# LeiXu84/fireFoam-dev

Measured on AMD Instinct MI355X. Metric: PIMPLE outer-iterations/sec on 64M-cell hex mesh; pEqn SpMV GB/s vs HBM peak, higher is better.
Workload: dtype f64; 1 GPU; synthetic 400^3 hex box (64000000 cells), buoyant plume + 5-species EDC-shaped source, PIMPLE 1/2/0: rhoEqn + UEqn + YEEqn(4 Yi + h) + 2 pEqn per step; cells=64000000, faces=191520000, parallelism=1 GPU, transport_solvers=PBiCGStab+DILU

## Files before the change

firefoam-dev_amd/binding.py:

```python
import ctypes as C
import os
import re
import subprocess

import numpy as np

_HERE = os.path.dirname(os.path.abspath(__file__))
_ROOT = os.path.dirname(_HERE)
_SO = os.path.join(_HERE, "lib", "libffm.so")
_HDR = os.path.join(_ROOT, "include", "ffm.h")

SOLVERS = {"PCG": 0, "PBiCGStab": 1, "PBiCG": 2, "diagonal": 3, "smoothSolver": 4}
PRECONDS = {"none": 0, "DIC": 1, "DILU": 2, "GaussSeidel": 3, "symGaussSeidel": 4, "diagonal": 5}


class FfmError(RuntimeError):
    pass


class Perf(C.Structure):
    _fields_ = [("initialResidual", C.c_double), ("finalResidual", C.c_double),
                ("nIterations", C.c_int), ("converged", C.c_int), ("singular", C.c_int)]

    def as_dict(self):
# ... 260 lines not shown
        "ffm_flow_order_create_staged": ([vp, C.POINTER(vp)], C.c_int),
        "ffm_flow_order_nstages": ([vp], C.c_int),
        "ffm_solve_ordered_staged_d": ([vp, vp, dp, dp, C.POINTER(Perf)], C.c_int),
        "ffm_plume_set_initial_state": ([vp, C.POINTER(C.c_void_p), hp, hp, hp, C.c_double], C.c_int),
        "ffm_plume_override_mv_weights": ([vp, hp], C.c_int),
        "ffm_plume_ncells": ([vp], C.c_int),
        "ffm_plume_nfaces": ([vp], C.c_int),
        "ffm_plume_get_field": ([vp, C.c_char_p, hp], C.c_int),
        "ffm_plume_nsolves": ([vp], C.c_int),
        "ffm_plume_joint_steps": ([vp], C.c_int),
        "ffm_plume_get_solve": ([vp, C.c_int, C.c_char_p, C.POINTER(Perf)], C.c_int),
        "ffm_plume_get_raw": ([vp, C.c_char_p, hp, C.c_long], C.c_long),
        "ffm_plume_ldu": ([vp], vp),
        "ffm_plume_mesh": ([vp], vp),
        "ffm_fv_multivariate_weights_tiled": ([vp, C.c_int, C.POINTER(C.c_int), C.c_double, C.c_double, C.c_double, dp] + [C.POINTER(C.c_void_p)] * 2 + [dp], C.c_int),
        "ffm_comm_unique_id": ([vp], C.c_int),
        "ffm_comm_init": ([vp, C.c_int, C.c_int, vp], C.c_int),
        "ffm_comm_init_host": ([vp, C.c_int, C.c_int, vp, HOST_ALLREDUCE_FN, HOST_EXCHANGE_FN], C.c_int),
        "ffm_comm_set_host_exchange2": ([vp, HOST_EXCHANGE2_FN], C.c_int),
        "ffm_plume_create_block": ([vp, C.c_int, C.c_int, C.c_int, ip, ip, ip, C.c_double, C.c_double, C.POINTER(vp)], C.c_int),
        "ffm_ldu_create_hint": ([vp, C.c_int, C.c_int, C.c_int, ip, ip, ip, C.POINTER(vp)], C.c_int),
        "ffm_renumber_hint": ([C.c_int, C.c_int, C.c_int, ip, ip, ip, ip, ip], C.c_int),
        "ffm_ldu_create_ext": ([vp, C.c_int, C.c_int, C.c_int, ip, ip, C.POINTER(vp)], C.c_int),
        "ffm_renumber_levels_ext": ([C.c_int, C.c_int, C.c_int, ip, ip, ip, ip], C.c_int),
        "ffm_ldu_check_layout": ([C.c_int, C.c_int, C.c_int, ip, ip], C.c_int),
        "ffm_ldu_set_ghost_exchange": ([vp, C.c_int, ip, ip, ip, ip], C.c_int),
        "ffm_halo_refresh_d": ([vp, dp], C.c_int),
        "ffm_ldu_nowned": ([vp], C.c_int),
        "ffm_comm_rank": ([vp], C.c_int),
        "ffm_comm_size": ([vp], C.c_int),
# ... 923 lines not shown
```

firefoam-dev_amd/csrc/ffm_fused.hip:

```cpp
#include "ffm_mesh.hpp"

constexpr int FUSE_MAX = 5;
constexpr int FUSE_MAX_OWN = 4;
#define CHECK_M(m) if (!(m)) { ffm_set_error("null mesh"); return FFM_ERR_ARG; }

struct GradMulti {
    const double *vf[FUSE_MAX], *vb[FUSE_MAX];
    double *gx[FUSE_MAX], *gy[FUSE_MAX], *gz[FUSE_MAX];
};

template <int W, int NF>
__global__ __launch_bounds__(256) void k_grad_multi(MeshView q, GradMulti a)
{
    CELL_SCHED(ci, q) {
        const int c = (int)ci;
        RowEnt<W> L, U; load_lower<W>(q.v, c, L); load_upper<W>(q.v, c, U);
        double wl[W], wu[W], sx[2 * W], sy[2 * W], sz[2 * W];
#pragma unroll
        for (int s = 0; s < W; s++) {
            wl[s] = q.w[L.f[s]]; wu[s] = q.w[U.f[s]];
            sx[s] = q.Sfx[L.f[s]]; sy[s] = q.Sfy[L.f[s]]; sz[s] = q.Sfz[L.f[s]];
            sx[W + s] = q.Sfx[U.f[s]]; sy[W + s] = q.Sfy[U.f[s]]; sz[W + s] = q.Sfz[U.f[s]];
        }
        const double V = q.V[c];
// ... 212 lines not shown
                        const int n = U.nb[s];
                        const double l = mv_limiter(sch, a.twoByk, a.lo, a.hi, fl[CH + s], vc, vf[n], dx[CH + s] * a.gx[i][n] + dy[CH + s] * a.gy[i][n] + dz[CH + s] * a.gz[i][n]);
                        lim[CH + s] = i == 0 ? l : fmin(lim[CH + s], l);
                    }
                }
            }
#pragma unroll
            for (int s = 0; s < CH; s++) {
                if (mine[s]) { const int e = L.f[s]; const double p0 = fl[s] >= 0 ? 1.0 : 0.0; a.out[e] = lim[s] * q.w[e] + (1.0 - lim[s]) * p0; }
                if (mine[CH + s] || ghostUp[s]) { const int e = U.f[s]; const double p0 = fl[CH + s] >= 0 ? 1.0 : 0.0; a.out[e] = lim[CH + s] * q.w[e] + (1.0 - lim[CH + s]) * p0; }
            }
        }
    }
}

constexpr int MVT_ENT = 256, MVT_FLD = 6, MVT_RUN = 32;
struct MvTile {
    const double *vf[MVT_FLD], *vb[MVT_FLD];
    int scheme[MVT_FLD], nf;
    const double *phi, *Cx, *Cy, *Cz;
    double twoByk, lo, hi;
    double *out;
    const int4 *seg, *rec;
};
template <int W>
__global__ __launch_bounds__(256) void k_mv_tile(MeshView q, MvTile a)
{
    __shared__ double ring[MVT_FLD][3 * MVT_ENT];
    __shared__ int4 shRec[3];
    const int4 sg = a.seg[blockIdx.x];
    const int gBeg = sg.x, ea = sg.y, eb = sg.z, gEnd = sg.w;
    const int t = threadIdx.x;
    const int nf = a.nf;
    auto stage = [&](int ee) {
        if (ee < gBeg || ee >= gEnd) { if (t == 0) shRec[(ee + 3) % 3] = make_int4(0, 0, 0, 0); return; }
        const int4 R = a.rec[ee];
        const int c0 = R.x, cnt = R.y & 0xFFFF;
        if (t == 0) shRec[ee % 3] = make_int4(c0, cnt, 0, 0);
        if (t < cnt) {
            const int c = c0 + t, o = (ee % 3) * MVT_ENT + t;
            for (int i = 0; i < nf; i++) ring[i][o] = a.vf[i][c];
        }
    };
    stage(ea - 1); stage(ea);
    for (int ee = ea; ee < eb; ee++) {
        stage(ee + 1);
        __syncthreads();
        const int4 Rm = shRec[(ee + 2) % 3], R0 = shRec[ee % 3], Rp = shRec[(ee + 1) % 3];
// ... 16 lines not shown
            }
            double gcur[2 * W];
#pragma unroll
            for (int s = 0; s < 2 * W; s++) gcur[s] = a.vf[0][gn[s]];
#pragma unroll
            for (int s = 0; s < W; s++) {
                fl[s] = L.on[s] ? a.phi[L.f[s]] : 0.0; mine[s] = L.on[s] && !(fl[s] > 0);
                fl[W + s] = U.on[s] ? a.phi[U.f[s]] : 0.0; mine[W + s] = U.on[s] && fl[W + s] > 0;
                lim[s] = lim[W + s] = 1.0;
                wl[s] = q.w[L.f[s]]; wu[s] = q.w[U.f[s]];
                sx[s] = q.Sfx[L.f[s]]; sy[s] = q.Sfy[L.f[s]]; sz[s] = q.Sfz[L.f[s]];
                sx[W + s] = q.Sfx[U.f[s]]; sy[W + s] = q.Sfy[U.f[s]]; sz[W + s] = q.Sfz[U.f[s]];
            }
#pragma unroll
            for (int s = 0; s < W; s++) {
                dx[s] = cx - a.Cx[L.nb[s]]; dy[s] = cy - a.Cy[L.nb[s]]; dz[s] = cz - a.Cz[L.nb[s]];
                dx[W + s] = a.Cx[U.nb[s]] - cx; dy[W + s] = a.Cy[U.nb[s]] - cy; dz[W + s] = a.Cz[U.nb[s]] - cz;
            }
            const double V = q.V[c];
            const int j = q.cellB[c];
#pragma unroll 1
            for (int i = 0; i < nf; i++) {
                const double P = ring[i][own];
                double vl[W], vu[W], gnext[2 * W];
                const double *__restrict__ vfn = a.vf[i + 1 < nf ? i + 1 : i];
#pragma unroll
                for (int s = 0; s < 2 * W; s++) gnext[s] = vfn[gn[s]];
#pragma unroll
                for (int s = 0; s < W; s++) {
                    const int k = sl[s] >= 0 ? sl[s] : own, ku = sl[W + s] >= 0 ? sl[W + s] : own;
                    const double rl = ring[i][k], ru = ring[i][ku];
                    vl[s] = sl[s] >= 0 ? rl : gcur[s]; vu[s] = sl[W + s] >= 0 ? ru : gcur[W + s];
// ... 3 lines not shown
                for (int s = 0; s < W; s++) if (L.on[s]) {
                    const double ff = wl[s] * vl[s] + (1.0 - wl[s]) * P;
                    ax -= sx[s] * ff; ay -= sy[s] * ff; az -= sz[s] * ff;
                }
#pragma unroll
                for (int s = 0; s < W; s++) if (U.on[s]) {
                    const double ff = wu[s] * P + (1.0 - wu[s]) * vu[s];
                    ax += sx[W + s] * ff; ay += sy[W + s] * ff; az += sz[W + s] * ff;
                }
                if (j >= 0) for (int tt = q.bcStart[j]; tt < q.bcStart[j + 1]; tt++) {
                    const int k = q.bcItem[tt]; const double b = a.vb[i][k];
                    ax += q.bSfx[k] * b; ay += q.bSfy[k] * b; az += q.bSfz[k] * b;
                }
                const double gxc = ax / V, gyc = ay / V, gzc = az / V;
                const int sch = a.scheme[i];
#pragma unroll
                for (int s = 0; s < W; s++) {
                    if (mine[s]) {
                        const double l = mv_limiter(sch, a.twoByk, a.lo, a.hi, fl[s], vl[s], P, dx[s] * gxc + dy[s] * gyc + dz[s] * gzc);
                        lim[s] = i == 0 ? l : fmin(lim[s], l);
                    }
                    if (mine[W + s]) {
                        const double l = mv_limiter(sch, a.twoByk, a.lo, a.hi, fl[W + s], P, vu[s], dx[W + s] * gxc + dy[W + s] * gyc + dz[W + s] * gzc);
                        lim[W + s] = i == 0 ? l : fmin(lim[W + s], l);
                    }
                }
#pragma unroll
                for (int s = 0; s < 2 * W; s++) gcur[s] = gnext[s];
            }
#pragma unroll
            for (int s = 0; s < W; s++) {
                if (mine[s]) { const int e = L.f[s]; const double p0 = fl[s] >= 0 ? 1.0 : 0.0; a.out[e] = lim[s] * q.w[e] + (1.0 - lim[s]) * p0; }
                if (mine[W + s]) { const int e = U.f[s]; const double p0 = fl[W + s] >= 0 ? 1.0 : 0.0; a.out[e] = lim[W + s] * q.w[e] + (1.0 - lim[W + s]) * p0; }
            }
        }
        __syncthreads();
    }
}

extern "C" int ffm_fv_multivariate_weights_tiled(ffm_mesh *m, int nf, const int *schemes, double k, double lo, double hi, const double *phi_f,
                                                 const double *const *vf, const double *const *vb, double *out_w)
{
    CHECK_M(m);
    if (nf < 1 || !schemes || !phi_f || !vf || !vb || !out_w) return FFM_ERR_ARG;
    FfmFvSegs sg;
    if (nf > MVT_FLD || m->A->maxW > 3 || !ffm_tile_fv_segments(m->A, MVT_RUN, &sg)) return FFM_ERR_UNSUPPORTED;
    MvTile a;
    for (int i = 0; i < MVT_FLD; i++) {
        const int qq = i < nf ? i : 0;
        if (i < nf && ((schemes[qq] != 2 && schemes[qq] != 3) || !vf[qq] || (m->B && !vb[qq]))) return FFM_ERR_ARG;
        a.vf[i] = vf[qq]; a.vb[i] = vb[qq]; a.scheme[i] = schemes[qq];
    }
    a.nf = nf; a.phi = phi_f; a.Cx = m->C[0]; a.Cy = m->C[1]; a.Cz = m->C[2]; a.twoByk = 2.0 / std::max(k, 1e-15); a.lo = lo; a.hi = hi; a.out = out_w;
    a.seg = sg.seg; a.rec = sg.rec;
    hipLaunchKernelGGL(k_mv_tile<3>, dim3(sg.nSeg), dim3(256), 0, m->ctx->stream, mview(m), a);
    FFM_HIP(hipGetLastError());
    return FFM_OK;
}

struct LustSource {
    const double *gx[3], *gy[3], *gz[3], *U0[3];
    double *src[3];
    const double *phi, *rho0, *Cx, *Cy, *Cz, *Cfx, *Cfy, *Cfz;
    double rdt;
};

template <int W>
__global__ __launch_bounds__(256) void k_lust_source(MeshView q, LustSource a)
{
    CELL_SCHED(ci, q) {
// ... 67 lines not shown
            const double w = limited_weight(a.scheme, a.twoByk, a.lo, a.hi, fl[s], wl[s], kl[s], P, dlx[s], dly[s], dlz[s], glx[s], gly[s], glz[s]);
            const double Kf = w * kl[s] + (1.0 - w) * P;
            acc = acc - fl[s] * Kf;
        }
#pragma unroll
        for (int s = 0; s < W; s++) if (U.on[s]) {
            const double w = limited_weight(a.scheme, a.twoByk, a.lo, a.hi, fu[s], wu[s], P, ku[s], dux[s], duy[s], duz[s], gux[s], guy[s], guz[s]);
            const double Kf = w * P + (1.0 - w) * ku[s];
            acc += fu[s] * Kf;
        }
        const int j = q.cellB[c];
        if (j >= 0) for (int t = q.bcStart[j]; t < q.bcStart[j + 1]; t++) { const int k = q.bcItem[t]; acc += a.phib[k] * a.Kb[k]; }
        a.divK[c] = acc / q.V[c];
        a.ddtK[c] = a.rdt * (a.rho[c] * P - a.rho0[c] * a.K0[c]);
        a.ndpdt[c] = -a.dpdt[c];
    }
}


extern "C" int ffm_fvc_grad_multi(ffm_mesh *m, int nf, const double *const *vf, const double *const *vb, double *const *gx,
                                  double *const *gy, double *const *gz)
{
    CHECK_M(m);
    if (nf < 1 || nf > FUSE_MAX_OWN || !vf || !vb || !gx || !gy || !gz) return FFM_ERR_ARG;
    GradMulti a;
    for (int i = 0; i < FUSE_MAX; i++) { const int k = i < nf ? i : 0; a.vf[i] = vf[k]; a.vb[i] = vb[k]; a.gx[i] = gx[k]; a.gy[i] = gy[k]; a.gz[i] = gz[k]; }
    for (int i = 0; i < nf; i++) if (!vf[i] || (m->B && !vb[i]) || !gx[i] || !gy[i] || !gz[i]) return FFM_ERR_ARG;
#define GM(NF) FFM_DISPATCH_W(m->A->maxW, LAUNCH_CELLS((k_grad_multi<W, NF>), mview(m), a))
    switch (nf) { case 1: GM(1); break; case 2: GM(2); break; case 3: GM(3); break; default: GM(4); break; }
#undef GM
// ... 169 lines not shown
    CHECK_M(m);
    if ((scheme != 2 && scheme != 3) || !phi_f || !K || !gx || !gy || !gz || !rho || !rho0 || !K0 || !dpdt || !divK || !ddtK || !negDpdt) return FFM_ERR_ARG;
    if (m->B && (!phi_b || !K_b)) return FFM_ERR_ARG;
    DivPhiK a;
    a.K = K; a.Kb = K_b; a.gx = gx; a.gy = gy; a.gz = gz; a.phi = phi_f; a.phib = phi_b; a.rho = rho; a.rho0 = rho0; a.K0 = K0; a.dpdt = dpdt;
    a.Cx = m->C[0]; a.Cy = m->C[1]; a.Cz = m->C[2]; a.divK = divK; a.ddtK = ddtK; a.ndpdt = negDpdt;
    a.rdt = rDeltaT; a.twoByk = 2.0 / std::max(k, 1e-15); a.lo = lo; a.hi = hi; a.scheme = scheme;
    if (m->A->maxW > 8) return FFM_ERR_UNSUPPORTED;
    if (m->A->maxW <= 3) LAUNCH_CELLS(k_div_phiK<3>, mview(m), a);
    else if (m->A->maxW <= 4) LAUNCH_CELLS(k_div_phiK<4>, mview(m), a);
    else LAUNCH_CELLS(k_div_phiK<8>, mview(m), a);
    FFM_HIP(hipGetLastError());
    return FFM_OK;
}

struct HbyA3 {
    const double *upper, *lower, *src[3], *ic[3], *bc[3], *psi[3], *rAU;
    double *out[3];
};
template <int W>
__global__ __launch_bounds__(256) void k_matrix_HbyA3(MeshView q, HbyA3 a)
{
    CELL_SCHED(ci, q) {
        const int c = (int)ci;
        RowEnt<W> L, U; load_lower<W>(q.v, c, L); load_upper<W>(q.v, c, U);
        double al[W], au[W];
#pragma unroll
        for (int s = 0; s < W; s++) { al[s] = a.lower[L.f[s]]; au[s] = a.upper[U.f[s]]; }
        double bd[3] = {0.0, 0.0, 0.0}, bda = 0.0, bs[3] = {0.0, 0.0, 0.0};
        const int j = q.cellB[c];
// ... 696 lines not shown
```

firefoam-dev_amd/csrc/ffm_plume.hip:

```cpp
#include "ffm_plume.hpp"

static int hydrostatic_init(ffm_plume *P)
{
    ffm_mesh *m = P->mesh; const int N = P->N, B = P->B;
    double *ph = P->ph_rgh, *rhof = P->wF[0], *sg = P->wF[1], *phig = P->wF[2], *rhob = P->wB[0], *fTop = P->wB[1], *div = P->wN[0];
    const double *gh = P->gh, *ghf = P->ghf, *magSf = ffm_mesh_geom(m, 1);
    double *p = P->p, *rho = P->rho; const double *psi = P->psi;
    const double *kind = P->kind_d;
    forN(P, B, [=] __device__(long k) { fTop[k] = (kind[k] > 1.5 && kind[k] < 2.5) ? 1.0 : 0.0; });
    forN(P, N, [=] __device__(long i) { p[i] = ph[i] + rho[i] * gh[i] + PREF; });
    FFM_TRY(thermo_correct(P)); mul(P, rho, psi, p, N);
    const long nNat = P->nNat;
    for (int corr = 0; corr < 5; corr++) {
        FFM_TRY(ffm_fvc_interpolate(m, nullptr, rho, rhof));
        zg(P, rhob, rho);
        FFM_TRY(ffm_fvc_snGrad(m, rho, sg));
        forN(P, nNat, [=] __device__(long e) { phig[e] = -rhof[e] * ghf[e] * sg[e] * magSf[e]; });
        FFM_TRY(ffm_fvm_transport(m, 0.0, nullptr, nullptr, nullptr, rhof, +1, P->diag, P->upper, P->lower));
        FFM_TRY(ffm_fvm_boundary_coeffs(m, nullptr, rhob, +1, fTop, P->zeroB, P->zeroB, P->ic[0], P->bc[0]));
        FFM_TRY(ffm_fvc_surface_integrate(m, phig, P->zeroB, div));
        {
            double *s0 = P->src[0]; const double *dv = div, *V = ffm_mesh_geom(m, 0);
            forN(P, N, [=] __device__(long i) { s0[i] = V[i] * dv[i]; });
        }
// ... 191 lines not shown
    P->fP = dalloc(P, B); P->refP = dalloc(P, B); P->gradP = dalloc(P, B); P->zeroB = dalloc(P, B);
    P->oneB = dupload(P, std::vector<double>(std::max(B, 1), 1.0));
    P->diag = NN(); P->upper = dalloc(P, nNat); P->lower = dalloc(P, nNat); P->dWork = NN(); P->sWork = NN();
    P->Udiag = NN(); P->Uupper = dalloc(P, nNat); P->Ulower = dalloc(P, nNat);
    for (int c = 0; c < 3; c++) { P->src[c] = NN(); P->ic[c] = dalloc(P, B); P->bc[c] = dalloc(P, B); P->Usrc[c] = NN(); P->Uic[c] = dalloc(P, B); P->Ubc[c] = dalloc(P, B); }
    for (auto &w : P->wN) w = NN();
    for (auto &w : P->wF) w = dalloc(P, nNat);
    P->ddtCorrF = dalloc(P, nNat);
    for (auto &w : P->wB) w = dalloc(P, B);
    for (int c = 0; c < 3; c++) { P->UdW[c] = NN(); P->UsW[c] = NN(); P->Ub[c] = P->wB[1 + c]; }
    P->wFuel = P->wN[8]; P->Qdot = P->wN[9]; P->Yt = P->wN[10]; P->alphaEff_f = P->wF[0]; P->alphaEff_b = P->wB[4];
    const bool fused = P->fused = getenv("FFM_PLUME_UNFUSED") == nullptr;
    P->mvSelection = getenv("FFM_PLUME_INDEPENDENT_LIMITERS") == nullptr;
    { const char *e = getenv("FFM_PLUME_SEPARATE_H"); P->separateH = e && atoi(e) != 0; }
    if (P->mvSelection) { P->wMv = dalloc(P, nNat); if (fused) for (int j = 0; j < 2; j++) for (int d = 0; d < 3; d++) P->mvG[j][d] = NN(); }
    for (int j = 0; j < 4; j++) {
        for (int d = 0; d < 3; d++) P->gM[j][d] = fused ? NN() : nullptr;
        P->spD[j] = fused ? NN() : nullptr; P->spS[j] = fused ? NN() : nullptr; P->suM[j] = fused ? NN() : nullptr;
        const bool ownOffDiag = fused && (j == 0 || !P->mvSelection);
        P->spU[j] = ownOffDiag ? dalloc(P, nNat) : nullptr; P->spL[j] = ownOffDiag ? dalloc(P, nNat) : nullptr; P->spB[j] = (fused || P->mvSelection) ? dalloc(P, B) : nullptr;
    }
    for (double *p : P->pool) if (!p) { ffm_set_error("plume: out of device memory"); return FFM_ERR_HIP; }
    PL_HIP(hipDeviceSynchronize());
    delete tmS_; tmS_ = new FfmStageTimer("plume_create: hydrostatic init");
    standin_thermo(P);
    mul(P, P->rho, P->psi, P->p, N);
    FFM_TRY(hydrostatic_init(P));
    PL_HIP(hipStreamSynchronize(ctx->stream));
    delete tmS_; tmS_ = nullptr;
    if (const char *e = getenv("FFM_PLUME_RADIATION")) { if (atoi(e) > 0) FFM_TRY(ffm_plume_set_radiation(P, atoi(e), 2, 4, nullptr, nullptr)); }
// ... 306 lines not shown
```

firefoam-dev_amd/csrc/ffm_plume.hpp:

```cpp
#pragma once
#include "ffm_internal.hpp"
#include "ffm_device.hpp"
#include <algorithm>
#include <cmath>
#include <string>

namespace {
constexpr double RR = 8314.47, CP = 1005.0, TREF = 298.15, PREF = 101325.0, MU = 1.8e-5, PR = 0.7;
constexpr double S_O2 = 3.6282945, HC = 46357151.0, TAU = 0.05, T_IN = 600.0, U_IN = 0.5, SIGMA_SB = 5.670367e-8;
constexpr int NSP = 5, INERT = 4;
const double WMOL[NSP] = {31.9988, 18.0153, 44.0962, 44.01, 28.0134};
const double Y_AMB[NSP] = {0.23301, 0.0, 0.0, 0.0, 0.76699};
const double Y_IN[NSP] = {0.0, 0.0, 1.0, 0.0, 0.0};
const double NU[NSP] = {-S_O2, 4 * 18.0153 / 44.0962, -1.0, 3 * 44.01 / 44.0962, 0.0};
const char *const SPN[NSP] = {"O2", "H2O", "C3H8", "CO2", "N2"};
enum { P_INLET = 0, P_FLOOR = 1, P_TOP = 2, P_SIDES = 3 };

template <class F> __global__ void k_for(long n, F f)
{
    for (long i = (long)blockIdx.x * blockDim.x + threadIdx.x; i < n; i += (long)gridDim.x * blockDim.x) f(i);
}
}

struct SolveLog { char name[16]; ffm_perf perf; };
// ... 9 lines not shown
    double hAmb = 0.0;
    std::vector<double *> pool;
    double *Y[NSP], *Y0[NSP], *T, *hs, *hs0, *U[3], *U0[3], *p, *p0, *p_rgh, *p_rgh0, *psi, *psi0, *rho, *rho0, *K, *K0, *dpdt;
    double *phi, *phib, *gh, *ghf, *ph_rgh, *ph_rgh_b;
    double *kind_d;
    double *fU[3], *refU[3], *fS, *refS, *fP, *refP, *gradP, *zeroB, *oneB;
    double *fStaticU[3], *fStaticS, *fStaticH, *fH, *refY[NSP], *refH;
    double *diag, *upper, *lower, *src[3], *ic[3], *bc[3], *dWork, *sWork;
    double *UdW[3], *UsW[3];
    double *wN[12], *wF[6], *wB[8];
    double *wFuel, *Qdot, *Yt, *alphaEff_f, *alphaEff_b, *Ub[3];
    double *ddtCorrF = nullptr; bool ddtCorrValid = false;
    double *gM[4][3], *spD[4], *spU[4], *spL[4], *spS[4], *spB[4], *suM[4];
    bool mvSelection = true;
    double *wMv = nullptr, *mvG[2][3] = {{nullptr, nullptr, nullptr}, {nullptr, nullptr, nullptr}};
    bool fused = true;
    bool separateH = false;
    int jointSteps = 0;
    double *Udiag, *Uupper, *Ulower, *Usrc[3], *Uic[3], *Ubc[3];
    std::vector<SolveLog> log;
    bool tight = false;
    int stepNo = 0, radFreq = 0;
    std::vector<double> rayD, rayOmega;
    std::vector<int> hL2, hU2, hOldToNew; std::vector<signed char> hFd2;
    int *radCm[3] = {nullptr, nullptr, nullptr}, *radFm[3] = {nullptr, nullptr, nullptr};
    double *radDB = nullptr, *radSB = nullptr, *radPsiB = nullptr, *radUB = nullptr, *radLB = nullptr;
    bool radOrdered = false;
    int radOrdering = 0; bool radMaps = false, radStaged = false;
    int nbrRank[6] = {-1, -1, -1, -1, -1, -1}, gOff[7] = {0, 0, 0, 0, 0, 0, 0}, blkGrid[3] = {1, 1, 1}, blkAt[3] = {0, 0, 0};
    int *radHaloCells = nullptr; int nRadHaloCells = 0; double *radGhostBuf = nullptr;
// ... 125 lines not shown
```

firefoam-dev_amd/csrc/ffm_plume_step.hip:

```cpp
#include "ffm_plume.hpp"

static void bc_update_f(ffm_plume *P, double *f, const double *fStatic)
{ const double *pb = P->phib; forN(P, P->B, [=] __device__(long k) { f[k] = fStatic[k] < 0 ? 1.0 - (pb[k] >= 0 ? 1.0 : 0.0) : fStatic[k]; }); }

static int update_bcs(ffm_plume *P)
{
    for (int c = 0; c < 3; c++) bc_update_f(P, P->fU[c], P->fStaticU[c]);
    bc_update_f(P, P->fS, P->fStaticS);
    bc_update_f(P, P->fH, P->fStaticH);
    return FFM_OK;
}

static int U_boundary(ffm_plume *P)
{
    for (int c = 0; c < 3; c++) FFM_TRY(ffm_bc_values(P->mesh, P->fU[c], P->refU[c], P->zeroB, P->U[c], P->Ub[c]));
    return FFM_OK;
}

static int bc_p_rgh(ffm_plume *P, const double *grad , const double *rhob)
{
    const double *kind = P->kind_d, *pb = P->phib, *phb = P->ph_rgh_b;
    const double *u0 = P->Ub[0], *u1 = P->Ub[1], *u2 = P->Ub[2];
    double *f = P->fP, *ref = P->refP, *g = P->gradP;
    forN(P, P->B, [=] __device__(long k) {
// ... 56 lines not shown
    { const double *phi = P->phi; forN(P, P->nNat, [=] __device__(long e) { corr[e] = phi[e] * corr[e]; }); }
    FFM_TRY(ffm_fvc_surface_integrate(m, corr, P->zeroB, divc));
    double *s = P->Usrc[c]; const double *rho0 = P->rho0, *u0 = P->U0[c];
    forN(P, P->N, [=] __device__(long i) { s[i] = rdt * rho0[i] * u0[i] * V[i] - V[i] * divc[i]; });
    return FFM_OK;
}
static int u_sources(ffm_plume *P, const double *mub)
{
    ffm_mesh *m = P->mesh; const bool ops = !P->fused;
    for (int c = 0; c < 3; c++) {
        FFM_TRY(ffm_fvm_boundary_coeffs(m, P->phib, mub, -1, P->fU[c], P->refU[c], P->zeroB, P->Uic[c], P->Ubc[c]));
        if (ops) FFM_TRY(u_source_ops(P, c));
    }
    if (ops) return FFM_OK;
    const double *uf[3] = {P->U[0], P->U[1], P->U[2]}, *ub[3] = {P->Ub[0], P->Ub[1], P->Ub[2]}, *u0[3] = {P->U0[0], P->U0[1], P->U0[2]};
    double *ggx[3] = {P->gM[0][0], P->gM[1][0], P->gM[2][0]}, *ggy[3] = {P->gM[0][1], P->gM[1][1], P->gM[2][1]}, *ggz[3] = {P->gM[0][2], P->gM[1][2], P->gM[2][2]};
    FFM_TRY(ffm_fvc_grad_multi(m, 3, uf, ub, ggx, ggy, ggz));
    for (int c = 0; c < 3; c++) { FFM_TRY(HX(P, ggx[c])); FFM_TRY(HX(P, ggy[c])); FFM_TRY(HX(P, ggz[c])); }
    return ffm_fvm_lust_source3(m, P->rdt, P->phi, P->rho0, u0, ggx, ggy, ggz, P->Usrc);
}

#define DIRECT_OR(P, direct, plain) \
    do { int rc_ = ((P)->oneBlock && ffm_tile_coef_direct_ok((P)->A)) ? (direct) : FFM_ERR_UNSUPPORTED; \
         if (rc_ == FFM_ERR_UNSUPPORTED) rc_ = (plain); FFM_TRY(rc_); } while (0)

static void les_gradU(ffm_plume *P, const double *g9[9])
{ for (int i = 0; i < 3; i++) for (int j = 0; j < 3; j++) g9[3 * i + j] = P->fused ? P->gM[j][i] : P->lesG[j][i]; }

static int les_rho_nuEff_faces(ffm_plume *P, double *gamCell, bool wantCell, double *rhob, double *gf, double *gb)
{
// ... 123 lines not shown

static int mv_weights_ops(ffm_plume *P, const MvFields &f)
{
    ffm_mesh *m = P->mesh;
    double *gx = P->wN[1], *gy = P->wN[2], *gz = P->wN[3], *lim = P->wF[1];
    for (int j = 0; j < 6; j++) {
        FFM_TRY(ffm_fvc_grad(m, f.vf[j], f.vb[j], gx, gy, gz));
        FFM_TRY(HX(P, gx)); FFM_TRY(HX(P, gy)); FFM_TRY(HX(P, gz));
        FFM_TRY(ffm_fv_limited_limiter(m, MV_SCHEMES[j], 1.0, 0.0, 1.0, P->phi, f.vf[j], gx, gy, gz, lim, j == 0 ? 0 : 1));
    }
    return ffm_fv_weights_from_limiter(m, P->phi, lim, P->wMv);
}

static int mv_weights(ffm_plume *P)
{
    if (!P->mvSelection) return FFM_OK;
    if (P->mvOverride) { P->mvOverride = false; return FFM_OK; }
    ffm_mesh *m = P->mesh;
    double *Nb = P->wB[1], *hb = P->wB[3];
    MvFields f = {{P->hs, nullptr, nullptr, nullptr, nullptr, P->Y[INERT]}, {hb, nullptr, nullptr, nullptr, nullptr, Nb}};
    for (int i = 0, j = 0; i < NSP; i++) if (i != INERT) {
        FFM_TRY(ffm_bc_values(m, P->fS, P->refY[i], P->zeroB, P->Y[i], P->spB[j]));
        f.vf[1 + j] = P->Y[i]; f.vb[1 + j] = P->spB[j]; j++;
    }
    {
        const double *b0 = P->spB[0], *b1 = P->spB[1], *b2 = P->spB[2], *b3 = P->spB[3];
        forN(P, P->B, [=] __device__(long k) { const double t = ((fmax(b0[k], 0.0) + fmax(b1[k], 0.0)) + fmax(b2[k], 0.0)) + fmax(b3[k], 0.0); Nb[k] = fmax(1.0 - t, 0.0); });
    }
    FFM_TRY(ffm_bc_values(m, P->fH, P->refH, P->zeroB, P->hs, hb));
    if (!P->fused) return mv_weights_ops(P, f);
    const int rc = ffm_fv_multivariate_weights_tiled(m, 6, MV_SCHEMES, 1.0, 0.0, 1.0, P->phi, f.vf, f.vb, P->wMv);
    return rc == FFM_ERR_UNSUPPORTED ? mv_weights_grad_multi(P, f) : rc;
}

static int scalar_transport(ffm_plume *P, const char *name, int scheme, double *vf, const double *vf0, const double *fBC, const double *ref,
                            const double *gamma_f, const double *gamma_b, const double *su, const double *const *expl, double tol,
                            const double *su2, const double *sp, const double *wGiven, const double *vbStored = nullptr)
{
    ffm_mesh *m = P->mesh; const int N = P->N;
    double *vb = P->wB[2], *gx = P->wN[1], *gy = P->wN[2], *gz = P->wN[3], *wOwn = P->wF[3], *sSu = P->wN[4];
    const double *w = wGiven;
    if (!wGiven) {
        if (!vbStored) FFM_TRY(ffm_bc_values(m, fBC, ref, P->zeroB, vf, vb));
        FFM_TRY(ffm_fvc_grad(m, vf, vbStored ? vbStored : vb, gx, gy, gz));
        FFM_TRY(HX(P, gx)); FFM_TRY(HX(P, gy)); FFM_TRY(HX(P, gz));
        FFM_TRY(ffm_fv_limited_weights(m, scheme, 1.0, 0.0, 1.0, P->phi, vf, gx, gy, gz, wOwn));
// ... 114 lines not shown
    ffm_mesh *m = P->mesh; const double rdt = P->rdt;
    double *wK = P->wF[3], *Kf = P->wF[4], *KfB = P->wB[5];
    FFM_TRY(ffm_fv_limited_weights(m, 2, 1.0, 0.0, 1.0, P->phi, P->K, kgx, kgy, kgz, wK));
    FFM_TRY(ffm_fvc_interpolate(m, wK, P->K, Kf));
    const double *phi = P->phi, *phib = P->phib;
    forN(P, P->nNat, [=] __device__(long e) { Kf[e] = phi[e] * Kf[e]; });
    forN(P, P->B, [=] __device__(long k) { KfB[k] = phib[k] * Kb[k]; });
    FFM_TRY(ffm_fvc_surface_integrate(m, Kf, KfB, kt.divK));
    const double *rho = P->rho, *rho0 = P->rho0, *K = P->K, *K0 = P->K0, *dpdt = P->dpdt; double *ddtK = kt.ddtK, *ndpdt = kt.ndpdt;
    forN(P, P->N, [=] __device__(long c) { ddtK[c] = rdt * (rho[c] * K[c] - rho0[c] * K0[c]); ndpdt[c] = -dpdt[c]; });
    return FFM_OK;
}
static int e_K_terms(ffm_plume *P, const KTerms &kt)
{
    ffm_mesh *m = P->mesh;
    double *Kb = P->wB[0], *kgx = P->wN[1], *kgy = P->wN[2], *kgz = P->wN[3];
    FFM_TRY(U_boundary(P));
    const double *b0 = P->Ub[0], *b1 = P->Ub[1], *b2 = P->Ub[2];
    forN(P, P->B, [=] __device__(long k) { Kb[k] = 0.5 * ((b0[k] * b0[k] + b1[k] * b1[k]) + b2[k] * b2[k]); });
    FFM_TRY(ffm_fvc_grad(m, P->K, Kb, kgx, kgy, kgz));
    FFM_TRY(HX(P, kgx)); FFM_TRY(HX(P, kgy)); FFM_TRY(HX(P, kgz));
    return P->fused ? ffm_fvc_div_phiK_terms(m, 2, 1.0, 0.0, 1.0, P->rdt, P->phi, P->phib, P->K, Kb, kgx, kgy, kgz, P->rho, P->rho0, P->K0, P->dpdt,
                                             kt.divK, kt.ddtK, kt.ndpdt)
                    : e_K_terms_ops(P, Kb, kgx, kgy, kgz, kt);
}

static int e_radiation_source(ffm_plume *P, const double **shSu, const double **shSp)
{
    *shSu = *shSp = nullptr;
    if (!(P->radCoupled && P->radHaveG)) return FFM_OK;
// ... 319 lines not shown
```

include/ffm.h:

```cpp
#ifndef FFM_H
#define FFM_H

#include <stddef.h>
#include <stdint.h>

#ifdef __cplusplus
extern "C" {
#endif

typedef struct ffm_ctx ffm_ctx;
typedef struct ffm_ldu ffm_ldu;

typedef enum ffm_status {
    FFM_OK = 0,
    FFM_ERR_ARG = -1,
    FFM_ERR_ADDR = -2,
    FFM_ERR_HIP = -3,
    FFM_ERR_NODEVICE = -4,
    FFM_ERR_UNSUPPORTED = -5,
    FFM_ERR_COMM = -6
} ffm_status;

typedef enum ffm_solver {
    FFM_PCG = 0, FFM_PBICGSTAB = 1, FFM_PBICG = 2, FFM_DIAGONAL = 3, FFM_SMOOTH = 4,
// ... 140 lines not shown
int ffm_fvc_surface_sum(ffm_mesh *m, const double *ssf_f, const double *ssf_b, double *out);
int ffm_fvc_grad(ffm_mesh *m, const double *vf, const double *vb, double *gx, double *gy, double *gz);
int ffm_fvc_reconstruct(ffm_mesh *m, const double *ssf_f, const double *ssf_b, double *ox, double *oy, double *oz);
int ffm_fvc_snGrad_correction(ffm_mesh *m, const double *gx, const double *gy, const double *gz, double *out_f);
int ffm_fv_limited_weights(ffm_mesh *m, int scheme, double k, double lo, double hi,
                           const double *phi_f, const double *vf, const double *gx,
                           const double *gy, const double *gz, double *out_w_f);
int ffm_fv_limited_limiter(ffm_mesh *m, int scheme, double k, double lo, double hi, const double *phi_f, const double *vf,
                           const double *gx, const double *gy, const double *gz, double *lim_f, int accumulateMin);
int ffm_fv_weights_from_limiter(ffm_mesh *m, const double *phi_f, const double *lim_f, double *out_w);
int ffm_fv_multivariate_weights(ffm_mesh *m, int nf, const int *schemes, double k, double lo, double hi, const double *phi_f,
                                const double *const *vf, const double *const *gx, const double *const *gy, const double *const *gz,
                                double *out_w);
int ffm_fv_multivariate_weights_tiled(ffm_mesh *m, int nf, const int *schemes, double k, double lo, double hi, const double *phi_f,
                                      const double *const *vf, const double *const *vb, double *out_w);

int ffm_fv_filtered_linear2V_weights(ffm_mesh *m, double k, double l, const double *phi_f, const double *const *U,
                                     const double *const *gx, const double *const *gy, const double *const *gz, double *out_w_f);

int ffm_fv_lust_correction(ffm_mesh *m, const double *phi_f, const double *gx, const double *gy,
                           const double *gz, double *out_f);
int ffm_fv_linear_upwind_correction(ffm_mesh *m, const double *phi_f, const double *gx, const double *gy,
                                    const double *gz, double *out_f);

int ffm_fvm_transport(ffm_mesh *m, double rDeltaT, const double *rho,
                      const double *phi_f, const double *w_f, const double *gamma_f,
                      int laplacianSign, double *diag, double *upper, double *lower);
int ffm_fvm_transport_scheme(ffm_mesh *m, double rDeltaT, const double *rho, const double *phi_f, int scheme,
                             const double *gamma_f, int laplacianSign, double *diag, double *upper, double *lower);
int ffm_fvm_transport_scheme_direct(ffm_mesh *m, double rDeltaT, const double *rho, const double *phi_f, int scheme,
// ... 292 lines not shown
```

Baseline: 3.269 outer-iterations/s.

## Fuse K-flux and LUST correction gradients into tiled multivariate kernel

Extends the tiled multivariate-weights kernel with a mode that also limits and interpolates kinetic energy K, writing phi*K face fluxes that a new cell-sum kernel turns into divK/ddtK. This replaces the separate K gradient, weights and divergence passes. A second mode computes the LUST velocity correction fluxes from in-tile gradients, followed by a cell-sum source kernel, instead of materialising full U gradients and running halo exchanges. Both aim to cut global memory traffic and kernel launches, at the cost of more shared memory, an extra ring field, and an extra face-sized buffer.

```diff
diff --git a/firefoam-dev_amd/binding.py b/firefoam-dev_amd/binding.py
--- a/firefoam-dev_amd/binding.py
+++ b/firefoam-dev_amd/binding.py
@@ -298,6 +298,11 @@
         "ffm_plume_ldu": ([vp], vp),
         "ffm_plume_mesh": ([vp], vp),
         "ffm_fv_multivariate_weights_tiled": ([vp, C.c_int, C.POINTER(C.c_int), C.c_double, C.c_double, C.c_double, dp] + [C.POINTER(C.c_void_p)] * 2 + [dp], C.c_int),
+        "ffm_fv_multivariate_weights_phiK_tiled": ([vp, C.c_int, C.POINTER(C.c_int), C.c_double, C.c_double, C.c_double, dp] + [C.POINTER(C.c_void_p)] * 2
+                                                   + [dp, C.c_int, C.c_double, C.c_double, C.c_double, dp, dp, dp], C.c_int),
+        "ffm_fvc_div_phiK_sum": ([vp, C.c_double] + [dp] * 11, C.c_int),
+        "ffm_fv_lust_phi_correction3_tiled": ([vp, dp] + [C.POINTER(C.c_void_p)] * 3, C.c_int),
+        "ffm_fvm_lust_source3_sum": ([vp, C.c_double, dp] + [C.POINTER(C.c_void_p)] * 3, C.c_int),
         "ffm_comm_unique_id": ([vp], C.c_int),
         "ffm_comm_init": ([vp, C.c_int, C.c_int, vp], C.c_int),
         "ffm_comm_init_host": ([vp, C.c_int, C.c_int, vp, HOST_ALLREDUCE_FN, HOST_EXCHANGE_FN], C.c_int),
diff --git a/firefoam-dev_amd/csrc/ffm_fused.hip b/firefoam-dev_amd/csrc/ffm_fused.hip
--- a/firefoam-dev_amd/csrc/ffm_fused.hip
+++ b/firefoam-dev_amd/csrc/ffm_fused.hip
@@ -250,7 +250,8 @@
     }
 }
 
-constexpr int MVT_ENT = 256, MVT_FLD = 6, MVT_RUN = 32;
+constexpr int MVT_ENT = 256, MVT_FLD = 7, MVT_RUN = 32;
+enum { MVT_W = 0, MVT_WK = 1, MVT_LUST = 2 };
 struct MvTile {
     const double *vf[MVT_FLD], *vb[MVT_FLD];
     int scheme[MVT_FLD], nf;
@@ -258,16 +259,20 @@
     double twoByk, lo, hi;
     double *out;
     const int4 *seg, *rec;
+    double kTwoByk, kLo, kHi;
+    const double *Cfx, *Cfy, *Cfz;
+    double *q[3];
 };
-template <int W>
+template <int W, int MODE>
 __global__ __launch_bounds__(256) void k_mv_tile(MeshView q, MvTile a)
 {
-    __shared__ double ring[MVT_FLD][3 * MVT_ENT];
+    constexpr int NRING = MODE == MVT_LUST ? 3 : MODE == MVT_WK ? MVT_FLD : MVT_FLD - 1;
+    __shared__ double ring[NRING][3 * MVT_ENT];
     __shared__ int4 shRec[3];
     const int4 sg = a.seg[blockIdx.x];
     const int gBeg = sg.x, ea = sg.y, eb = sg.z, gEnd = sg.w;
     const int t = threadIdx.x;
-    const int nf = a.nf;
+    const int nf = MODE == MVT_LUST ? 3 : MODE == MVT_WK ? a.nf + 1 : a.nf;
     auto stage = [&](int ee) {
         if (ee < gBeg || ee >= gEnd) { if (t == 0) shRec[(ee + 3) % 3] = make_int4(0, 0, 0, 0); return; }
         const int4 R = a.rec[ee];
@@ -314,8 +319,13 @@
             }
 #pragma unroll
             for (int s = 0; s < W; s++) {
-                dx[s] = cx - a.Cx[L.nb[s]]; dy[s] = cy - a.Cy[L.nb[s]]; dz[s] = cz - a.Cz[L.nb[s]];
-                dx[W + s] = a.Cx[U.nb[s]] - cx; dy[W + s] = a.Cy[U.nb[s]] - cy; dz[W + s] = a.Cz[U.nb[s]] - cz;
+                if (MODE == MVT_LUST) {
+                    dx[s] = a.Cfx[L.f[s]] - cx; dy[s] = a.Cfy[L.f[s]] - cy; dz[s] = a.Cfz[L.f[s]] - cz;
+                    dx[W + s] = a.Cfx[U.f[s]] - cx; dy[W + s] = a.Cfy[U.f[s]] - cy; dz[W + s] = a.Cfz[U.f[s]] - cz;
+                } else {
+                    dx[s] = cx - a.Cx[L.nb[s]]; dy[s] = cy - a.Cy[L.nb[s]]; dz[s] = cz - a.Cz[L.nb[s]];
+                    dx[W + s] = a.Cx[U.nb[s]] - cx; dy[W + s] = a.Cy[U.nb[s]] - cy; dz[W + s] = a.Cz[U.nb[s]] - cz;
+                }
             }
             const double V = q.V[c];
             const int j = q.cellB[c];
@@ -349,24 +359,51 @@
                 }
                 const double gxc = ax / V, gyc = ay / V, gzc = az / V;
                 const int sch = a.scheme[i];
-#pragma unroll
-                for (int s = 0; s < W; s++) {
-                    if (mine[s]) {
-                        const double l = mv_limiter(sch, a.twoByk, a.lo, a.hi, fl[s], vl[s], P, dx[s] * gxc + dy[s] * gyc + dz[s] * gzc);
-                        lim[s] = i == 0 ? l : fmin(lim[s], l);
+                if (MODE == MVT_LUST) {
+                    double *__restrict__ qi = a.q[i];
+#pragma unroll
+                    for (int s = 0; s < 2 * W; s++) if (mine[s]) {
+                        const double corr = 0.25 * ((dx[s] * gxc + dy[s] * gyc) + dz[s] * gzc);
+                        qi[s < W ? L.f[s] : U.f[s - W]] = fl[s] * corr;
                     }
-                    if (mine[W + s]) {
-                        const double l = mv_limiter(sch, a.twoByk, a.lo, a.hi, fl[W + s], P, vu[s], dx[W + s] * gxc + dy[W + s] * gyc + dz[W + s] * gzc);
-                        lim[W + s] = i == 0 ? l : fmin(lim[W + s], l);
+                } else if (MODE == MVT_WK && i == nf - 1) {
+#pragma unroll
+                    for (int s = 0; s < W; s++) {
+                        if (mine[s]) {
+                            const double l = mv_limiter(sch, a.kTwoByk, a.kLo, a.kHi, fl[s], vl[s], P, dx[s] * gxc + dy[s] * gyc + dz[s] * gzc);
+                            const double p0 = fl[s] >= 0 ? 1.0 : 0.0, w = l * wl[s] + (1.0 - l) * p0;
+                            const double Kf = w * vl[s] + (1.0 - w) * P;
+                            a.q[0][L.f[s]] = fl[s] * Kf;
+                        }
+                        if (mine[W + s]) {
+                            const double l = mv_limiter(sch, a.kTwoByk, a.kLo, a.kHi, fl[W + s], P, vu[s], dx[W + s] * gxc + dy[W + s] * gyc + dz[W + s] * gzc);
+                            const double p0 = fl[W + s] >= 0 ? 1.0 : 0.0, w = l * wu[s] + (1.0 - l) * p0;
+                            const double Kf = w * P + (1.0 - w) * vu[s];
+                            a.q[0][U.f[s]] = fl[W + s] * Kf;
+                        }
+                    }
+                } else {
+#pragma unroll
+                    for (int s = 0; s < W; s++) {
+                        if (mine[s]) {
+                            const double l = mv_limiter(sch, a.twoByk, a.lo, a.hi, fl[s], vl[s], P, dx[s] * gxc + dy[s] * gyc + dz[s] * gzc);
+                            lim[s] = i == 0 ? l : fmin(lim[s], l);
+                        }
+                        if (mine[W + s]) {
+                            const double l = mv_limiter(sch, a.twoByk, a.lo, a.hi, fl[W + s], P, vu[s], dx[W + s] * gxc + dy[W + s] * gyc + dz[W + s] * gzc);
+                            lim[W + s] = i == 0 ? l : fmin(lim[W + s], l);
+                        }
                     }
                 }
 #pragma unroll
                 for (int s = 0; s < 2 * W; s++) gcur[s] = gnext[s];
             }
-#pragma unroll
-            for (int s = 0; s < W; s++) {
-                if (mine[s]) { const int e = L.f[s]; const double p0 = fl[s] >= 0 ? 1.0 : 0.0; a.out[e] = lim[s] * q.w[e] + (1.0 - lim[s]) * p0; }
-                if (mine[W + s]) { const int e = U.f[s]; const double p0 = fl[W + s] >= 0 ? 1.0 : 0.0; a.out[e] = lim[W + s] * q.w[e] + (1.0 - lim[W + s]) * p0; }
+            if (MODE != MVT_LUST) {
+#pragma unroll
+                for (int s = 0; s < W; s++) {
+                    if (mine[s]) { const int e = L.f[s]; const double p0 = fl[s] >= 0 ? 1.0 : 0.0; a.out[e] = lim[s] * q.w[e] + (1.0 - lim[s]) * p0; }
+                    if (mine[W + s]) { const int e = U.f[s]; const double p0 = fl[W + s] >= 0 ? 1.0 : 0.0; a.out[e] = lim[W + s] * q.w[e] + (1.0 - lim[W + s]) * p0; }
+                }
             }
         }
         __syncthreads();
@@ -379,8 +416,8 @@
     CHECK_M(m);
     if (nf < 1 || !schemes || !phi_f || !vf || !vb || !out_w) return FFM_ERR_ARG;
     FfmFvSegs sg;
-    if (nf > MVT_FLD || m->A->maxW > 3 || !ffm_tile_fv_segments(m->A, MVT_RUN, &sg)) return FFM_ERR_UNSUPPORTED;
-    MvTile a;
+    if (nf > MVT_FLD - 1 || m->A->maxW > 3 || !ffm_tile_fv_segments(m->A, MVT_RUN, &sg)) return FFM_ERR_UNSUPPORTED;
+    MvTile a = {};
     for (int i = 0; i < MVT_FLD; i++) {
         const int qq = i < nf ? i : 0;
         if (i < nf && ((schemes[qq] != 2 && schemes[qq] != 3) || !vf[qq] || (m->B && !vb[qq]))) return FFM_ERR_ARG;
@@ -388,7 +425,49 @@
     }
     a.nf = nf; a.phi = phi_f; a.Cx = m->C[0]; a.Cy = m->C[1]; a.Cz = m->C[2]; a.twoByk = 2.0 / std::max(k, 1e-15); a.lo = lo; a.hi = hi; a.out = out_w;
     a.seg = sg.seg; a.rec = sg.rec;
-    hipLaunchKernelGGL(k_mv_tile<3>, dim3(sg.nSeg), dim3(256), 0, m->ctx->stream, mview(m), a);
+    hipLaunchKernelGGL((k_mv_tile<3, MVT_W>), dim3(sg.nSeg), dim3(256), 0, m->ctx->stream, mview(m), a);
+    FFM_HIP(hipGetLastError());
+    return FFM_OK;
+}
+
+extern "C" int ffm_fv_multivariate_weights_phiK_tiled(ffm_mesh *m, int nf, const int *schemes, double k, double lo, double hi, const double *phi_f,
+                                                      const double *const *vf, const double *const *vb, double *out_w, int schemeK, double kK,
+                                                      double loK, double hiK, const double *K, const double *K_b, double *out_phiK)
+{
+    CHECK_M(m);
+    if (nf < 1 || !schemes || !phi_f || !vf || !vb || !out_w || (schemeK != 2 && schemeK != 3) || !K || (m->B && !K_b) || !out_phiK) return FFM_ERR_ARG;
+    FfmFvSegs sg;
+    if (nf > MVT_FLD - 1 || m->A->maxW > 3 || !ffm_tile_fv_segments(m->A, MVT_RUN, &sg)) return FFM_ERR_UNSUPPORTED;
+    MvTile a = {};
+    for (int i = 0; i < MVT_FLD; i++) {
+        const int qq = i < nf ? i : 0;
+        if (i < nf && ((schemes[qq] != 2 && schemes[qq] != 3) || !vf[qq] || (m->B && !vb[qq]))) return FFM_ERR_ARG;
+        a.vf[i] = vf[qq]; a.vb[i] = vb[qq]; a.scheme[i] = schemes[qq];
+    }
+    a.vf[nf] = K; a.vb[nf] = K_b; a.scheme[nf] = schemeK;
+    a.nf = nf; a.phi = phi_f; a.Cx = m->C[0]; a.Cy = m->C[1]; a.Cz = m->C[2]; a.twoByk = 2.0 / std::max(k, 1e-15); a.lo = lo; a.hi = hi; a.out = out_w;
+    a.kTwoByk = 2.0 / std::max(kK, 1e-15); a.kLo = loK; a.kHi = hiK; a.q[0] = out_phiK;
+    a.seg = sg.seg; a.rec = sg.rec;
+    hipLaunchKernelGGL((k_mv_tile<3, MVT_WK>), dim3(sg.nSeg), dim3(256), 0, m->ctx->stream, mview(m), a);
+    FFM_HIP(hipGetLastError());
+    return FFM_OK;
+}
+
+extern "C" int ffm_fv_lust_phi_correction3_tiled(ffm_mesh *m, const double *phi_f, const double *const *U, const double *const *U_b,
+                                                 double *const *out_q)
+{
+    CHECK_M(m);
+    if (!phi_f || !U || !U_b || !out_q) return FFM_ERR_ARG;
+    FfmFvSegs sg;
+    if (m->A->maxW > 3 || !ffm_tile_fv_segments(m->A, MVT_RUN, &sg)) return FFM_ERR_UNSUPPORTED;
+    if (!m->Cf[0]) { ffm_set_error("ffm_fv_lust_phi_correction3_tiled: face centres not set (ffm_mesh_set_face_centres)"); return FFM_ERR_ARG; }
+    MvTile a = {};
+    for (int i = 0; i < 3; i++) if (!U[i] || (m->B && !U_b[i]) || !out_q[i]) return FFM_ERR_ARG;
+    for (int i = 0; i < MVT_FLD; i++) { a.vf[i] = U[i < 3 ? i : 0]; a.vb[i] = U_b[i < 3 ? i : 0]; }
+    for (int i = 0; i < 3; i++) a.q[i] = out_q[i];
+    a.nf = 3; a.phi = phi_f; a.Cx = m->C[0]; a.Cy = m->C[1]; a.Cz = m->C[2]; a.Cfx = m->Cf[0]; a.Cfy = m->Cf[1]; a.Cfz = m->Cf[2];
+    a.seg = sg.seg; a.rec = sg.rec;
+    hipLaunchKernelGGL((k_mv_tile<3, MVT_LUST>), dim3(sg.nSeg), dim3(256), 0, m->ctx->stream, mview(m), a);
     FFM_HIP(hipGetLastError());
     return FFM_OK;
 }
@@ -486,6 +565,63 @@
         a.divK[c] = acc / q.V[c];
         a.ddtK[c] = a.rdt * (a.rho[c] * P - a.rho0[c] * a.K0[c]);
         a.ndpdt[c] = -a.dpdt[c];
+    }
+}
+
+struct PhiKSum {
+    const double *qf, *Kb, *phib, *K, *rho, *rho0, *K0, *dpdt;
+    double *divK, *ddtK, *ndpdt;
+    double rdt;
+};
+template <int W>
+__global__ __launch_bounds__(256) void k_phiK_sum(MeshView q, PhiKSum a)
+{
+    CELL_SCHED(ci, q) {
+        const int c = (int)ci;
+        RowEnt<W> L, U; load_lower<W>(q.v, c, L); load_upper<W>(q.v, c, U);
+        double ql[W], qu[W];
+#pragma unroll
+        for (int s = 0; s < W; s++) { ql[s] = a.qf[L.f[s]]; qu[s] = a.qf[U.f[s]]; }
+        double acc = 0.0;
+#pragma unroll
+        for (int s = 0; s < W; s++) if (L.on[s]) acc = acc - ql[s];
+#pragma unroll
+        for (int s = 0; s < W; s++) if (U.on[s]) acc += qu[s];
+        const int j = q.cellB[c];
+        if (j >= 0) for (int t = q.bcStart[j]; t < q.bcStart[j + 1]; t++) { const int k = q.bcItem[t]; acc += a.phib[k] * a.Kb[k]; }
+        a.divK[c] = acc / q.V[c];
+        a.ddtK[c] = a.rdt * (a.rho[c] * a.K[c] - a.rho0[c] * a.K0[c]);
+        a.ndpdt[c] = -a.dpdt[c];
+    }
+}
+
+struct LustSum {
+    const double *qf[3], *U0[3];
+    double *src[3];
+    const double *rho0;
+    double rdt;
+};
+template <int W>
+__global__ __launch_bounds__(256) void k_lust_sum(MeshView q, LustSum a)
+{
+    CELL_SCHED(ci, q) {
+        const int c = (int)ci;
+        RowEnt<W> L, U; load_lower<W>(q.v, c, L); load_upper<W>(q.v, c, U);
+        const double V = q.V[c], r0 = a.rho0[c];
+#pragma unroll
+        for (int i = 0; i < 3; i++) {
+            const double *__restrict__ qf = a.qf[i];
+            double ql[W], qu[W];
+#pragma unroll
+            for (int s = 0; s < W; s++) { ql[s] = qf[L.f[s]]; qu[s] = qf[U.f[s]]; }
+            double acc = 0.0;
+#pragma unroll
+            for (int s = 0; s < W; s++) if (L.on[s]) acc -= ql[s];
+#pragma unroll
+            for (int s = 0; s < W; s++) if (U.on[s]) acc += qu[s];
+            const double divc = acc / V;
+            a.src[i][c] = a.rdt * r0 * a.U0[i][c] * V - V * divc;
+        }
     }
 }
 
@@ -685,6 +821,36 @@
     return FFM_OK;
 }
 
+extern "C" int ffm_fvc_div_phiK_sum(ffm_mesh *m, double rDeltaT, const double *phiK_f, const double *phi_b, const double *K, const double *K_b,
+                                    const double *rho, const double *rho0, const double *K0, const double *dpdt, double *divK, double *ddtK,
+                                    double *negDpdt)
+{
+    CHECK_M(m);
+    if (!phiK_f || !K || !rho || !rho0 || !K0 || !dpdt || !divK || !ddtK || !negDpdt || (m->B && (!phi_b || !K_b))) return FFM_ERR_ARG;
+    PhiKSum a;
+    a.qf = phiK_f; a.Kb = K_b; a.phib = phi_b; a.K = K; a.rho = rho; a.rho0 = rho0; a.K0 = K0; a.dpdt = dpdt;
+    a.divK = divK; a.ddtK = ddtK; a.ndpdt = negDpdt; a.rdt = rDeltaT;
+    FFM_DISPATCH_W(m->A->maxW, LAUNCH_CELLS(k_phiK_sum<W>, mview(m), a));
+    FFM_HIP(hipGetLastError());
+    return FFM_OK;
+}
+
+extern "C" int ffm_fvm_lust_source3_sum(ffm_mesh *m, double rDeltaT, const double *rho0, const double *const *U0, const double *const *q_f,
+                                        double *const *source)
+{
+    CHECK_M(m);
+    if (!rho0 || !U0 || !q_f || !source) return FFM_ERR_ARG;
+    LustSum a;
+    for (int i = 0; i < 3; i++) {
+        if (!U0[i] || !q_f[i] || !source[i]) return FFM_ERR_ARG;
+        a.qf[i] = q_f[i]; a.U0[i] = U0[i]; a.src[i] = source[i];
+    }
+    a.rho0 = rho0; a.rdt = rDeltaT;
+    FFM_DISPATCH_W(m->A->maxW, LAUNCH_CELLS(k_lust_sum<W>, mview(m), a));
+    FFM_HIP(hipGetLastError());
+    return FFM_OK;
+}
+
 struct HbyA3 {
     const double *upper, *lower, *src[3], *ic[3], *bc[3], *psi[3], *rAU;
     double *out[3];
diff --git a/firefoam-dev_amd/csrc/ffm_plume.hip b/firefoam-dev_amd/csrc/ffm_plume.hip
--- a/firefoam-dev_amd/csrc/ffm_plume.hip
+++ b/firefoam-dev_amd/csrc/ffm_plume.hip
@@ -229,6 +229,7 @@
     P->mvSelection = getenv("FFM_PLUME_INDEPENDENT_LIMITERS") == nullptr;
     { const char *e = getenv("FFM_PLUME_SEPARATE_H"); P->separateH = e && atoi(e) != 0; }
     if (P->mvSelection) { P->wMv = dalloc(P, nNat); if (fused) for (int j = 0; j < 2; j++) for (int d = 0; d < 3; d++) P->mvG[j][d] = NN(); }
+    if (P->mvSelection && fused && P->oneBlock) { P->phiKf = dalloc(P, nNat); P->KbM = dalloc(P, B); }
     for (int j = 0; j < 4; j++) {
         for (int d = 0; d < 3; d++) P->gM[j][d] = fused ? NN() : nullptr;
         P->spD[j] = fused ? NN() : nullptr; P->spS[j] = fused ? NN() : nullptr; P->suM[j] = fused ? NN() : nullptr;
diff --git a/firefoam-dev_amd/csrc/ffm_plume.hpp b/firefoam-dev_amd/csrc/ffm_plume.hpp
--- a/firefoam-dev_amd/csrc/ffm_plume.hpp
+++ b/firefoam-dev_amd/csrc/ffm_plume.hpp
@@ -47,6 +47,7 @@
     double *gM[4][3], *spD[4], *spU[4], *spL[4], *spS[4], *spB[4], *suM[4];
     bool mvSelection = true;
     double *wMv = nullptr, *mvG[2][3] = {{nullptr, nullptr, nullptr}, {nullptr, nullptr, nullptr}};
+    double *phiKf = nullptr, *KbM = nullptr; bool phiKValid = false;
     bool fused = true;
     bool separateH = false;
     int jointSteps = 0;
diff --git a/firefoam-dev_amd/csrc/ffm_plume_step.hip b/firefoam-dev_amd/csrc/ffm_plume_step.hip
--- a/firefoam-dev_amd/csrc/ffm_plume_step.hip
+++ b/firefoam-dev_amd/csrc/ffm_plume_step.hip
@@ -94,6 +94,12 @@
     }
     if (ops) return FFM_OK;
     const double *uf[3] = {P->U[0], P->U[1], P->U[2]}, *ub[3] = {P->Ub[0], P->Ub[1], P->Ub[2]}, *u0[3] = {P->U0[0], P->U0[1], P->U0[2]};
+    if (P->oneBlock && !P->turbModel) {
+        double *qf[3] = {P->wF[1], P->wF[2], P->wF[4]};
+        const int rc = ffm_fv_lust_phi_correction3_tiled(m, P->phi, uf, ub, qf);
+        if (rc == FFM_OK) return ffm_fvm_lust_source3_sum(m, P->rdt, P->rho0, u0, qf, P->Usrc);
+        if (rc != FFM_ERR_UNSUPPORTED) return rc;
+    }
     double *ggx[3] = {P->gM[0][0], P->gM[1][0], P->gM[2][0]}, *ggy[3] = {P->gM[0][1], P->gM[1][1], P->gM[2][1]}, *ggz[3] = {P->gM[0][2], P->gM[1][2], P->gM[2][2]};
     FFM_TRY(ffm_fvc_grad_multi(m, 3, uf, ub, ggx, ggy, ggz));
     for (int c = 0; c < 3; c++) { FFM_TRY(HX(P, ggx[c])); FFM_TRY(HX(P, ggy[c])); FFM_TRY(HX(P, ggz[c])); }
@@ -247,9 +253,16 @@
 
 static int mv_weights(ffm_plume *P)
 {
+    P->phiKValid = false;
     if (!P->mvSelection) return FFM_OK;
     if (P->mvOverride) { P->mvOverride = false; return FFM_OK; }
     ffm_mesh *m = P->mesh;
+    const bool withK = P->fused && P->oneBlock && P->phiKf;
+    if (withK) {
+        FFM_TRY(U_boundary(P));
+        double *Kb = P->KbM; const double *b0 = P->Ub[0], *b1 = P->Ub[1], *b2 = P->Ub[2];
+        forN(P, P->B, [=] __device__(long k) { Kb[k] = 0.5 * ((b0[k] * b0[k] + b1[k] * b1[k]) + b2[k] * b2[k]); });
+    }
     double *Nb = P->wB[1], *hb = P->wB[3];
     MvFields f = {{P->hs, nullptr, nullptr, nullptr, nullptr, P->Y[INERT]}, {hb, nullptr, nullptr, nullptr, nullptr, Nb}};
     for (int i = 0, j = 0; i < NSP; i++) if (i != INERT) {
@@ -262,7 +275,10 @@
     }
     FFM_TRY(ffm_bc_values(m, P->fH, P->refH, P->zeroB, P->hs, hb));
     if (!P->fused) return mv_weights_ops(P, f);
-    const int rc = ffm_fv_multivariate_weights_tiled(m, 6, MV_SCHEMES, 1.0, 0.0, 1.0, P->phi, f.vf, f.vb, P->wMv);
+    const int rc = withK ? ffm_fv_multivariate_weights_phiK_tiled(m, 6, MV_SCHEMES, 1.0, 0.0, 1.0, P->phi, f.vf, f.vb, P->wMv, 2, 1.0, 0.0, 1.0, P->K,
+                                                                  P->KbM, P->phiKf)
+                         : ffm_fv_multivariate_weights_tiled(m, 6, MV_SCHEMES, 1.0, 0.0, 1.0, P->phi, f.vf, f.vb, P->wMv);
+    if (rc == FFM_OK) P->phiKValid = withK;
     return rc == FFM_ERR_UNSUPPORTED ? mv_weights_grad_multi(P, f) : rc;
 }
 
@@ -407,6 +423,8 @@
 static int e_K_terms(ffm_plume *P, const KTerms &kt)
 {
     ffm_mesh *m = P->mesh;
+    if (P->phiKValid)
+        return ffm_fvc_div_phiK_sum(m, P->rdt, P->phiKf, P->phib, P->K, P->KbM, P->rho, P->rho0, P->K0, P->dpdt, kt.divK, kt.ddtK, kt.ndpdt);
     double *Kb = P->wB[0], *kgx = P->wN[1], *kgy = P->wN[2], *kgz = P->wN[3];
     FFM_TRY(U_boundary(P));
     const double *b0 = P->Ub[0], *b1 = P->Ub[1], *b2 = P->Ub[2];
diff --git a/include/ffm.h b/include/ffm.h
--- a/include/ffm.h
+++ b/include/ffm.h
@@ -178,6 +178,16 @@
                                 double *out_w);
 int ffm_fv_multivariate_weights_tiled(ffm_mesh *m, int nf, const int *schemes, double k, double lo, double hi, const double *phi_f,
                                       const double *const *vf, const double *const *vb, double *out_w);
+int ffm_fv_multivariate_weights_phiK_tiled(ffm_mesh *m, int nf, const int *schemes, double k, double lo, double hi, const double *phi_f,
+                                           const double *const *vf, const double *const *vb, double *out_w, int schemeK, double kK,
+                                           double loK, double hiK, const double *K, const double *K_b, double *out_phiK);
+int ffm_fvc_div_phiK_sum(ffm_mesh *m, double rDeltaT, const double *phiK_f, const double *phi_b, const double *K, const double *K_b,
+                         const double *rho, const double *rho0, const double *K0, const double *dpdt, double *divK, double *ddtK,
+                         double *negDpdt);
+int ffm_fv_lust_phi_correction3_tiled(ffm_mesh *m, const double *phi_f, const double *const *U, const double *const *U_b,
+                                      double *const *out_q);
+int ffm_fvm_lust_source3_sum(ffm_mesh *m, double rDeltaT, const double *rho0, const double *const *U0, const double *const *q_f,
+                             double *const *source);
 
 int ffm_fv_filtered_linear2V_weights(ffm_mesh *m, double k, double l, const double *phi_f, const double *const *U,
                                      const double *const *gx, const double *const *gy, const double *const *gz, double *out_w_f);
```

Result: faster. 3.336 outer-iterations/s (median of 6 runs) (+2.0%).
